# SDFIdk/malstroem

Measured on AMD Instinct MI355X. Metric: Mcells/s fill->D8->accum->label on 16384^2 f32 DEM, higher is better.
Workload: dtype f32 fill / f64 no-flats+D8+accum / u8 flowdir / i32 labels; 1 GPU; 16384x16384 float32 DEM (spectral fBm beta=2 seed 42 (SURVEY 8d recipe)): fill+depths -> no-flats fill -> D8 -> accumulation -> CCL+label_stats -> watersheds+label_count -> pour points; parallelism=1 GPU, one device context, fill_rounds=9, noflat_rounds=84, fill_tiles=70225, fill_visits=44601, fill_cycles=0, noflat_visits=411396, noflat_cycles=411396, nlabels=4637017, fill_algorithm=1, fill_launches=9, noflat_algorithm=2, pour_algorithm=1

## Files before the change

### malstroem_amd/csrc/watershed.hip

```cpp
#include <algorithm>

#include <type_traits>

#include "common.hpp"

namespace mh {
namespace {

constexpr int32_t NONE = 0x7fffffff;
constexpr uint32_t QFLAG = 0x80000000u, QMASK = 0x7fffffffu, QTERM = 0x7fffffffu;

__global__ __launch_bounds__(256) void ws_count_interior_nodir(const uint8_t *__restrict__ fd, int64_t H, int64_t W,
                                                              unsigned int *count)
{
    const int64_t i0 = ((int64_t)blockIdx.x * blockDim.x + threadIdx.x) * 16, n = H * W;
    unsigned hits = 0;
    if (i0 < n) {
        int64_t r = i0 / W, c = i0 - r * W;
        uint8_t b[16];
        const bool whole = i0 + 16 <= n;
        if (whole) {
            *reinterpret_cast<uint4 *>(b) = *reinterpret_cast<const uint4 *>(fd + i0);
        } else {
#pragma unroll
            for (int k = 0; k < 16; ++k) b[k] = i0 + k < n ? fd[i0 + k] : (uint8_t)0;
        }
#pragma unroll
        for (int k = 0; k < 16; ++k) {
            hits += (b[k] > 7u && r > 0 && r < H - 1 && c > 0 && c < W - 1) ? 1u : 0u;
            if (++c == W) {
                c = 0;
                ++r;
            }
        }
    }
#pragma unroll
    for (int o = 32; o > 0; o >>= 1) hits += __shfl_xor(hits, o);
    if (hits && (threadIdx.x & 63) == 0) atomicAdd(count, hits);
}

__global__ __launch_bounds__(256) void ws_init_kernel(const uint8_t *__restrict__ fd, const int32_t *__restrict__ lab,
                                                     int32_t *__restrict__ P, uint32_t *__restrict__ Q, int64_t H, int64_t W,
                                                     int32_t unassigned)
{
    const int64_t i = (int64_t)blockIdx.x * blockDim.x + threadIdx.x;
    if (i >= H * W) return;
    const int64_t d = downstream(fd, i, H, W);
    P[i] = lab[i] != unassigned ? (int32_t)i : (d < 0 ? NONE : (int32_t)d);
    if (Q) {
        const int64_t r = i / W, c = i - r * W;
        const bool edge = r == 0 || r == H - 1 || c == 0 || c == W - 1;
        Q[i] = (edge ? QFLAG : 0u) | (d < 0 ? QTERM : (uint32_t)d);
    }
}

constexpr int HOPS = 5;
constexpr int32_t DONE = (int32_t)0x80000000;
__global__ __launch_bounds__(256) void ws_jump_kernel(int32_t *P, uint32_t *Q, int64_t n, unsigned int *open)
{
    const int64_t i = (int64_t)blockIdx.x * blockDim.x + threadIdx.x;
    if (i >= n) return;
    bool ch = false;
    int32_t t = P[i];
    if (t >= 0 && t != NONE && t != (int32_t)i) {
        const int32_t t0 = t;
#pragma unroll
        for (int h = 0; h < HOPS; ++h) {
            const int32_t pt = P[t];
            if (pt == t) {
                t |= DONE;
                break;
            }
            t = pt;
            if (t < 0 || t == NONE) break;
        }
        if (t != t0) P[i] = t;
        ch = t >= 0 && t != NONE;
    }
    if (Q) {
        uint32_t q = Q[i];
        const uint32_t q0 = q;
#pragma unroll
        for (int h = 0; h < HOPS; ++h) {
            const uint32_t idx = q & QMASK;
            if (idx == QTERM) break;
            const uint32_t qt = Q[idx];
            q = ((q | qt) & QFLAG) | (qt & QMASK);
        }
        if (q != q0) Q[i] = q;
        ch |= (q & QMASK) != QTERM;
    }
    if (ch) *open = 1u;
}

constexpr int WT = WS_TILE;
__global__ __launch_bounds__(256) void ws_tile_kernel(const uint8_t *__restrict__ fd, const int32_t *__restrict__ lab, int32_t *__restrict__ P, int64_t H,
                                                     int64_t W, int ntc, int32_t unassigned, PourCandDev pc, int32_t *__restrict__ Pn)
{
    __shared__ uint16_t ptr[WT * WT];
    __shared__ uint8_t val[WT * WT];
    constexpr uint8_t V_LAB = 8, V_NONE = 9;
    const int ti = blockIdx.x / ntc, tj = blockIdx.x - ti * ntc;
    const int64_t r0 = (int64_t)ti * WT, c0 = (int64_t)tj * WT;
    const int lr = threadIdx.x >> 2, lc0 = (threadIdx.x & 3) * 16;
    const int64_t r = r0 + lr, cbase = c0 + lc0;
    const bool vec = (W & 15) == 0 && r < H && cbase + 16 <= W;
    uint8_t code[16];
    int32_t lb[16];
    if (vec) {
        const uint4 cv = *reinterpret_cast<const uint4 *>(fd + r * W + cbase);
        memcpy(code, &cv, 16);
#pragma unroll
        for (int q = 0; q < 4; ++q) {
            const int4 lv = *reinterpret_cast<const int4 *>(lab + r * W + cbase + 4 * q);
            lb[4 * q] = lv.x; lb[4 * q + 1] = lv.y; lb[4 * q + 2] = lv.z; lb[4 * q + 3] = lv.w;
        }
    } else {
#pragma unroll
        for (int k = 0; k < 16; ++k) {
            const bool in = r < H && cbase + k < W;
            code[k] = in ? fd[r * W + cbase + k] : (uint8_t)8;
            lb[k] = in ? lab[r * W + cbase + k] : unassigned;
        }
    }
    uint32_t lmask = 0;
    auto init_cells = [&](auto inner_tag) {
        constexpr bool INNER = decltype(inner_tag)::value;
#pragma unroll
        for (int k = 0; k < 16; ++k) {
            const int li = lr * WT + lc0 + k;
            const int64_t c = cbase + k;
            uint16_t p = (uint16_t)li;
            uint8_t v = V_NONE;
            if (INNER || (r < H && c < W)) {
                if (lb[k] != unassigned) {
                    lmask |= 1u << k;
                    v = V_LAB;
                } else if (code[k] <= 7u) {
                    const int lr2 = lr + dir_dr((int)code[k]), lc2 = lc0 + k + dir_dc((int)code[k]);
                    bool in_raster = true;
                    if (!INNER) {
                        const int64_t nr = r0 + lr2, nc = c0 + lc2;
                        in_raster = nr >= 0 && nr < H && nc >= 0 && nc < W;
                    }
                    if (in_raster) {
                        if (lr2 >= 0 && lr2 < WT && lc2 >= 0 && lc2 < WT) p = (uint16_t)(lr2 * WT + lc2);
                        else v = code[k];
                    }
                }
            }
            ptr[li] = p;
            val[li] = v;
        }
    };
    if (r0 > 0 && c0 > 0 && r0 + WT < H && c0 + WT < W) init_cells(std::true_type{});
    else init_cells(std::false_type{});
    __syncthreads();
    if (pc.mask0) {
        uint32_t cw[4] = {0x08080808u, 0x08080808u, 0x08080808u, 0x08080808u};
        if (vec) {
            const uint4 cv = *reinterpret_cast<const uint4 *>(fd + r * W + cbase);
            cw[0] = cv.x; cw[1] = cv.y; cw[2] = cv.z; cw[3] = cv.w;
        } else {
#pragma unroll
            for (int k = 0; k < 16; ++k)
                if (r < H && cbase + k < W) cw[k >> 2] = (cw[k >> 2] & ~(0xffu << (8 * (k & 3)))) | ((uint32_t)fd[r * W + cbase + k] << (8 * (k & 3)));
        }
        const uint32_t Wu = (uint32_t)W, Hu = (uint32_t)H, r0u = (uint32_t)r0, c0u = (uint32_t)c0;
        uint32_t m0 = 0, ml = 0;
#pragma unroll
        for (int k = 0; k < 16; ++k) {
            if (!(r < H && cbase + k < W)) continue;
            const unsigned cd = (cw[k >> 2] >> (8 * (k & 3))) & 0xffu;
            const bool mylab = (lmask >> k) & 1u;
            bool same = false;
            if (cd <= 7u) {
                const int lr2 = lr + dir_dr((int)cd), lc2 = lc0 + k + dir_dc((int)cd);
                const uint32_t nr = r0u + (uint32_t)lr2, nc = c0u + (uint32_t)lc2;
                if (nr < Hu && nc < Wu) {
                    const uint32_t gd = nr * Wu + nc;
                    bool labelled_d;
                    if (lr2 >= 0 && lr2 < WT && lc2 >= 0 && lc2 < WT) labelled_d = val[lr2 * WT + lc2] == V_LAB;
                    else labelled_d = lab[gd] != unassigned;
                    if (pc.components) same = labelled_d == mylab;
                    else same = (labelled_d ? lab[gd] : unassigned) == (mylab ? lab[(uint32_t)(r * W + cbase + k)] : unassigned);
                }
            }
            if (!same) {
                if (!mylab) m0 |= 1u << k;
                else ml |= 1u << k;
            }
        }
        pc.mask0[(int64_t)blockIdx.x * 256 + threadIdx.x] = (uint16_t)m0;
        __shared__ uint32_t wsum[4], base_s;
        const int lane = threadIdx.x & 63, wave = threadIdx.x >> 6;
        const uint32_t mine = (uint32_t)__builtin_popcount(ml);
        uint32_t incl = mine;
#pragma unroll
        for (int o = 1; o < 64; o <<= 1) {
            const uint32_t up = (uint32_t)__shfl_up((int)incl, o);
            if (lane >= o) incl += up;
        }
        if (lane == 63) wsum[wave] = incl;
        __syncthreads();
        if (threadIdx.x == 0) {
            const uint32_t tot = wsum[0] + wsum[1] + wsum[2] + wsum[3];
            const bool fits = tot <= POUR_TILE_CAP;
            if (!fits) pc.flags[0] = 1u;
            pc.tile_cnt[blockIdx.x] = fits ? tot : 0u;
            base_s = fits ? blockIdx.x * POUR_TILE_CAP : 0xffffffffu;
        }
        __syncthreads();
        if (base_s != 0xffffffffu) {
            uint32_t o = base_s + incl - mine;
            for (int w = 0; w < wave; ++w) o += wsum[w];
#pragma unroll
            for (int k = 0; k < 16; ++k)
                if ((ml >> k) & 1u) {
                    const uint32_t cell = (uint32_t)(r * W + cbase + k);
                    pc.list[o++] = make_uint2(cell, (uint32_t)lab[cell]);
                }
        }
    }
    for (int round = 0; round < 13; ++round) {
        bool ch = false;
#pragma unroll
        for (int k = 0; k < 16; ++k) {
            const int li = k * 256 + (int)threadIdx.x;
            const uint16_t p = ptr[li], q = ptr[p];
            if (q != p) {
                ptr[li] = q;
                ch = true;
            }
        }
        if (!__syncthreads_or(ch)) break;
    }
    int32_t out[16];
#pragma unroll
    for (int k = 0; k < 16; ++k) {
        const int li = lr * WT + lc0 + k;
        const int t = ptr[li];
        const int64_t gt = (r0 + (t >> 6)) * W + c0 + (t & 63);
        if (ptr[t] != t) out[k] = (int32_t)gt;
        else {
            const unsigned vb = val[t];
            int32_t v = NONE;
            if (vb == V_LAB) v = (int32_t)gt;
            else if (vb <= 7u) v = (int32_t)((r0 + (t >> 6) + dir_dr((int)vb)) * W + c0 + (t & 63) + dir_dc((int)vb));
            out[k] = (vb == V_LAB && t != li) ? (v | DONE) : v;
        }
        const int slot = ws_perim_slot(lr, lc0 + k);
        if (slot >= 0) Pn[(int64_t)blockIdx.x * 256 + slot] = (r < H && cbase + k < W) ? out[k] : NONE;
    }
    if (vec) {
#pragma unroll
        for (int q = 0; q < 4; ++q) *reinterpret_cast<int4 *>(P + r * W + cbase + 4 * q) = make_int4(out[4 * q], out[4 * q + 1], out[4 * q + 2], out[4 * q + 3]);
    } else {
#pragma unroll
        for (int k = 0; k < 16; ++k)
            if (r < H && cbase + k < W) P[r * W + cbase + k] = out[k];
    }
}

__global__ __launch_bounds__(256) void ws_jump_perimeter_kernel(int32_t *Pn, int64_t W, int ntc, int64_t nnodes, unsigned int *open)
{
    const int64_t x = (int64_t)blockIdx.x * blockDim.x + threadIdx.x;
    if (x >= nnodes || (x & 255) >= 4 * WT - 4) return;
    int32_t t = Pn[x];
    if (t < 0 || t == NONE) return;
    if (ws_node_of(t, (uint32_t)W, ntc) == x) return;
    const int32_t t0 = t;
#pragma unroll
    for (int h = 0; h < HOPS; ++h) {
        const int64_t nd = ws_node_of(t, (uint32_t)W, ntc);
        if (nd < 0) {
            if (t != t0) Pn[x] = t;
            return;
        }
        const int32_t pt = Pn[nd];
        if (pt == t) {
            t |= DONE;
            break;
        }
        t = pt;
        if (t < 0 || t == NONE) break;
    }
    if (t != t0) Pn[x] = t;
    if (t >= 0 && t != NONE) *open = 1u;
}

__global__ __launch_bounds__(256) void ws_assign_hop_kernel(const int32_t *__restrict__ P, const int32_t *__restrict__ Pn, const int32_t *src, int32_t *lab, int64_t n,
                                                           int64_t W, int ntc)
{
    const int64_t i0 = ((int64_t)blockIdx.x * blockDim.x + threadIdx.x) * 4;
    if (i0 >= n) return;
    const bool copy = src != lab;
    auto target = [&](int64_t i, int32_t p) -> int32_t {
        if (p == NONE || p == (int32_t)i) return -1;
        if (p >= 0) {
            const int64_t nd = ws_node_of(p, (uint32_t)W, ntc);
            if (nd < 0) return -1;
            const int32_t q = Pn[nd];
            if (q == p) p = q | DONE;
            else if (q < 0) p = q;
            else return -1;
        }
        return p & ~DONE;
    };
    if (i0 + 4 <= n && copy) {
        const int4 p4 = *reinterpret_cast<const int4 *>(P + i0);
        int4 v = *reinterpret_cast<const int4 *>(src + i0);
        const int32_t pq[4] = {p4.x, p4.y, p4.z, p4.w};
        int64_t nd[4];
        int32_t q[4], t[4];
#pragma unroll
        for (int k = 0; k < 4; ++k) {
            const bool hop = pq[k] >= 0 && pq[k] != NONE && pq[k] != (int32_t)(i0 + k);
            nd[k] = hop ? ws_node_of(pq[k], (uint32_t)W, ntc) : -1;
        }
#pragma unroll
        for (int k = 0; k < 4; ++k) q[k] = nd[k] >= 0 ? Pn[nd[k]] : NONE;
#pragma unroll
        for (int k = 0; k < 4; ++k) {
            int32_t pp = pq[k];
            t[k] = -1;
            if (pp == NONE || pp == (int32_t)(i0 + k)) continue;
            if (pp >= 0) {
                if (nd[k] < 0) continue;
                if (q[k] == pp) pp = q[k] | DONE;
                else if (q[k] < 0) pp = q[k];
                else continue;
            }
            t[k] = pp & ~DONE;
        }
        int32_t lv[4];
#pragma unroll
        for (int k = 0; k < 4; ++k) lv[k] = src[t[k] >= 0 ? t[k] : 0];
        if (t[0] >= 0) v.x = lv[0];
        if (t[1] >= 0) v.y = lv[1];
        if (t[2] >= 0) v.z = lv[2];
        if (t[3] >= 0) v.w = lv[3];
        *reinterpret_cast<int4 *>(lab + i0) = v;
    } else if (i0 + 4 <= n) {
        const int4 p = *reinterpret_cast<const int4 *>(P + i0);
        const int32_t t0 = target(i0, p.x), t1 = target(i0 + 1, p.y), t2 = target(i0 + 2, p.z), t3 = target(i0 + 3, p.w);
        if (copy) {
            int4 v = *reinterpret_cast<const int4 *>(src + i0);
            if (t0 >= 0) v.x = src[t0];
            if (t1 >= 0) v.y = src[t1];
            if (t2 >= 0) v.z = src[t2];
            if (t3 >= 0) v.w = src[t3];
            *reinterpret_cast<int4 *>(lab + i0) = v;
        } else {
            if (t0 >= 0) lab[i0] = src[t0];
            if (t1 >= 0) lab[i0 + 1] = src[t1];
            if (t2 >= 0) lab[i0 + 2] = src[t2];
            if (t3 >= 0) lab[i0 + 3] = src[t3];
        }
    } else {
        for (int64_t i = i0; i < n; ++i) {
            const int32_t t = target(i, P[i]);
            if (t >= 0) lab[i] = src[t];
            else if (copy) lab[i] = src[i];
        }
    }
}

__global__ __launch_bounds__(256) void ws_assign_kernel(const int32_t *__restrict__ P, const uint32_t *__restrict__ Q,
                                                       int32_t *lab, int64_t n, int32_t unassigned)
{
    const int64_t i = (int64_t)blockIdx.x * blockDim.x + threadIdx.x;
    if (i >= n) return;
    const int32_t p = P[i];
    if (p >= 0) return;
    const int32_t t = p & ~DONE;
    if (Q && !(Q[t] & QFLAG)) return;
    lab[i] = lab[t];
}

__global__ void ws_pseudo_kernel(int32_t *ws, int64_t H, int64_t W, int top, int bottom)
{
    const int64_t c = (int64_t)blockIdx.x * blockDim.x + threadIdx.x;
    if (c >= W) return;
    if (top) ws[c] = -(int32_t)(1 + c);
    if (bottom) ws[(H - 1) * W + c] = -(int32_t)(1 + W + c);
}
__global__ __launch_bounds__(256) void ws_root_labels_kernel(int32_t *out, int64_t H, int64_t W, int64_t row_off, int64_t Hg)
{
    const int64_t i = (int64_t)blockIdx.x * blockDim.x + threadIdx.x;
    if (i >= H * W) return;
    const int64_t r = i / W, c = i - r * W, gr = r + row_off;
    out[i] = (gr == 0 || gr == Hg - 1 || c == 0 || c == W - 1) ? BAND_ROOT : 0;
}
__global__ __launch_bounds__(256) void ws_hide_rootless_kernel(const int32_t *__restrict__ lab, const int32_t *__restrict__ rooted,
                                                              int32_t *__restrict__ out, int64_t n)
{
    const int64_t i = (int64_t)blockIdx.x * blockDim.x + threadIdx.x;
    if (i >= n) return;
    const int32_t l = lab[i];
    out[i] = (l == 0 || rooted[i] == BAND_ROOT) ? l : BAND_ROOTLESS;
}
__global__ __launch_bounds__(256) void ws_show_rootless_kernel(int32_t *__restrict__ ws, const int32_t *__restrict__ lab, int64_t n)
{
    const int64_t i = (int64_t)blockIdx.x * blockDim.x + threadIdx.x;
    if (i < n && ws[i] == BAND_ROOTLESS) ws[i] = lab[i];
}
__global__ __launch_bounds__(256) void ws_neg_lut_kernel(int32_t *lab, int64_t n, const int32_t *__restrict__ lut, int64_t nlut)
{
    const int64_t i0 = ((int64_t)blockIdx.x * blockDim.x + threadIdx.x) * 4;
    if (i0 >= n) return;
    auto look = [&](int32_t v) -> int32_t { return (v < 0 && (int64_t)(-(int64_t)v - 1) < nlut) ? lut[-(int64_t)v - 1] : v; };
    if (i0 + 4 <= n) {
        const int4 v = *reinterpret_cast<const int4 *>(lab + i0);
        if ((v.x | v.y | v.z | v.w) >= 0) return;
        *reinterpret_cast<int4 *>(lab + i0) = make_int4(look(v.x), look(v.y), look(v.z), look(v.w));
    } else {
        for (int64_t i = i0; i < n; ++i) lab[i] = look(lab[i]);
    }
}

}

int band_pseudo_labels_dev(int32_t *d_ws, int64_t H, int64_t W, int top, int bottom, hipStream_t s)
{
    hipLaunchKernelGGL(ws_pseudo_kernel, dim3((unsigned)cdiv(W, 256)), dim3(256), 0, s, d_ws, H, W, top, bottom);
    MH_HIP(hipGetLastError());
    return MHIP_OK;
}

int band_root_labels_dev(int32_t *d_out, int64_t H, int64_t W, int64_t row_off, int64_t Hg, hipStream_t s)
{
    hipLaunchKernelGGL(ws_root_labels_kernel, dim3((unsigned)cdiv(H * W, 256)), dim3(256), 0, s, d_out, H, W, row_off, Hg);
    MH_HIP(hipGetLastError());
    return MHIP_OK;
}

int band_hide_rootless_dev(const int32_t *d_lab, const int32_t *d_rooted, int32_t *d_out, int64_t n, hipStream_t s)
{
    hipLaunchKernelGGL(ws_hide_rootless_kernel, dim3((unsigned)cdiv(n, 256)), dim3(256), 0, s, d_lab, d_rooted, d_out, n);
    MH_HIP(hipGetLastError());
    return MHIP_OK;
}

int band_show_rootless_dev(int32_t *d_ws, const int32_t *d_lab, int64_t n, hipStream_t s)
{
    hipLaunchKernelGGL(ws_show_rootless_kernel, dim3((unsigned)cdiv(n, 256)), dim3(256), 0, s, d_ws, d_lab, n);
    MH_HIP(hipGetLastError());
    return MHIP_OK;
}

int negative_lut_dev(int32_t *d_lab, int64_t n, const int32_t *d_lut, int64_t nlut, hipStream_t s)
{
    hipLaunchKernelGGL(ws_neg_lut_kernel, dim3((unsigned)cdiv(cdiv(n, 4), 256)), dim3(256), 0, s, d_lab, n, d_lut, nlut);
    MH_HIP(hipGetLastError());
    return MHIP_OK;
}

namespace {
__global__ __launch_bounds__(1024) void pour_key0_kernel(const unsigned long long *__restrict__ tile_key0, int64_t ntiles, unsigned long long *key)
{
    unsigned long long best = 0;
    for (int64_t t = (int64_t)blockIdx.x * 1024 + threadIdx.x; t < ntiles; t += (int64_t)gridDim.x * 1024) best = tile_key0[t] > best ? tile_key0[t] : best;
#pragma unroll
    for (int o = 32; o > 0; o >>= 1) {
        const unsigned long long ob = __shfl_xor(best, o);
        best = ob > best ? ob : best;
    }
    if ((threadIdx.x & 63) == 0 && best) atomicMax(&key[0], best);
}

__global__ __launch_bounds__(256) void pour_finish_kernel(const unsigned long long *__restrict__ key, int64_t nrec, int64_t W, mhip_index_record *rec)
{
    const int64_t i = (int64_t)blockIdx.x * blockDim.x + threadIdx.x;
    if (i >= nrec) return;
    mhip_index_record r;
    const unsigned long long k = key[i];
    if (k == 0) {
        r.value = -__builtin_inf();
        r.row = -1;
        r.col = -1;
    } else {
        const uint64_t p = 0xffffffffu - (uint32_t)k;
        r.value = (double)(uint32_t)(k >> 32);
        r.row = (int64_t)(p / (uint64_t)W);
        r.col = (int64_t)(p % (uint64_t)W);
    }
    rec[i] = r;
}

}

int pour_finish_dev(unsigned long long *d_key, const unsigned long long *d_tile_key0, int64_t ntiles, int64_t nlab, int64_t W, mhip_index_record *d_rec,
                    hipStream_t s)
{
    hipLaunchKernelGGL(pour_key0_kernel, dim3((unsigned)std::min<int64_t>(cdiv(ntiles, 1024), 64)), dim3(1024), 0, s, d_tile_key0, ntiles, d_key);
    hipLaunchKernelGGL(pour_finish_kernel, dim3((unsigned)cdiv(nlab + 1, 256)), dim3(256), 0, s, d_key, nlab + 1, W, d_rec);
    MH_HIP(hipGetLastError());
    return MHIP_OK;
}

namespace {
struct PourNotify {
    PourLink *pl;
    bool done = false;
    void operator()(int v)
    {
        if (pl && pl->notify && !done) pl->notify(pl->arg, v);
        done = true;
    }
    ~PourNotify() { (*this)(0); }
};
}

int watersheds_dev(const uint8_t *d_fd, int32_t *d_labels, int64_t H, int64_t W, int32_t unassigned, hipStream_t s, bool band_mode,
                   const unsigned int *d_known_interior_nodir, const int32_t *d_src, PourLink *pour)
{
    PourNotify notify{pour};
    const int32_t *src = d_src ? d_src : d_labels;
    const int64_t n = H * W;
    if (n >= (int64_t)NONE - 1) {
        set_error("watersheds: %lld cells exceed the int32 index domain", (long long)n);
        return MHIP_ELIMIT;
    }
    const unsigned grid = (unsigned)cdiv(n, 256);
    DevBuf P, Q, flags;
    MH_TRY(P.alloc(4 * (size_t)n));
    MH_TRY(flags.alloc(sizeof(unsigned int) * 4));
    MH_HIP(hipMemsetAsync(flags.p, 0, sizeof(unsigned int) * 4, s));
    unsigned int *d_cnt = flags.as<unsigned int>(), *d_changed = d_cnt + 2;
    unsigned int interior_nodir = 0;
    if (!d_known_interior_nodir) hipLaunchKernelGGL(ws_count_interior_nodir, dim3((unsigned)cdiv(cdiv(n, 16), 256)), dim3(256), 0, s, d_fd, H, W, d_cnt);
    MH_HIP(hipMemcpyAsync(&interior_nodir, d_known_interior_nodir ? d_known_interior_nodir : d_cnt, 4, hipMemcpyDeviceToHost, s));
    MH_HIP(stream_sync(s));
    uint32_t *q = nullptr;
    if (interior_nodir && band_mode) {
        set_error("watersheds on a row band in one local pass need every flow path to leave the raster (interior NODIR cell found): "
                  "mhip_ctx_band_watershed_rooted takes any flow directions");
        return MHIP_EINVAL;
    }
    if (interior_nodir || (!d_known_interior_nodir && !band_mode)) {
        MH_TRY(Q.alloc(4 * (size_t)n));
        q = Q.as<uint32_t>();
    }
    if (!q) {
        const int64_t ntr = cdiv(H, WT), ntc = cdiv(W, WT), ntiles = ntr * ntc;
        const bool cand = pour && pour->dev.mask0 && unassigned == 0 && n < 0xffffffffll;
        DevBuf Pn;
        MH_TRY(Pn.alloc(4 * 256 * (size_t)ntiles));
        hipLaunchKernelGGL(ws_tile_kernel, dim3((unsigned)ntiles), dim3(256), 0, s, d_fd, src, P.as<int32_t>(), H, W, (int)ntc, unassigned,
                           cand ? pour->dev : PourCandDev(), Pn.as<int32_t>());
        if (cand) {
            MH_HIP(hipEventRecord(pour->ev, s));
            notify(1);
        } else {
            notify(0);
        }
        constexpr int MAX_ROUNDS = 40;
        for (int round = 0; round < MAX_ROUNDS;) {
            const int k = round == 0 ? 2 : 1;
            MH_HIP(hipMemsetAsync(d_changed, 0, 8, s));
            for (int j = 0; j < k; ++j)
                hipLaunchKernelGGL(ws_jump_perimeter_kernel, dim3((unsigned)ntiles), dim3(256), 0, s, Pn.as<int32_t>(), W, (int)ntc, ntiles * 256, d_changed + j);
            unsigned int h[2] = {0, 0};
            MH_HIP(hipMemcpyAsync(h, d_changed, 8, hipMemcpyDeviceToHost, s));
            MH_HIP(stream_sync(s));
            round += k;
            if (!h[k - 1]) break;
        }
        hipLaunchKernelGGL(ws_assign_hop_kernel, dim3((unsigned)cdiv(cdiv(n, 4), 256)), dim3(256), 0, s, P.as<int32_t>(), Pn.as<int32_t>(), src, d_labels, n, W,
                           (int)ntc);
        MH_HIP(hipGetLastError());
        MH_HIP(stream_sync(s));
        return MHIP_OK;
    }
    if (src != d_labels) MH_HIP(hipMemcpyAsync(d_labels, src, 4 * (size_t)n, hipMemcpyDeviceToDevice, s));
    hipLaunchKernelGGL(ws_init_kernel, dim3(grid), dim3(256), 0, s, d_fd, d_labels, P.as<int32_t>(), q, H, W, unassigned);
    constexpr int MAX_ROUNDS = 32;
    for (int round = 0; round < MAX_ROUNDS;) {
        const int k = round == 0 ? 2 : 1;
        MH_HIP(hipMemsetAsync(d_changed, 0, 8, s));
        for (int j = 0; j < k; ++j)
            hipLaunchKernelGGL(ws_jump_kernel, dim3(grid), dim3(256), 0, s, P.as<int32_t>(), q, n, d_changed + j);
        unsigned int h[2] = {0, 0};
        MH_HIP(hipMemcpyAsync(h, d_changed, 8, hipMemcpyDeviceToHost, s));
        MH_HIP(stream_sync(s));
        round += k;
        if (!h[k - 1]) break;
    }
    hipLaunchKernelGGL(ws_assign_kernel, dim3(grid), dim3(256), 0, s, P.as<int32_t>(), q, d_labels, n, unassigned);
    MH_HIP(hipGetLastError());
    MH_HIP(stream_sync(s));
    return MHIP_OK;
}

}
```

Measured before the change: 12350 Mcells/s.

## Restructure watershed tile kernel: byte-offset pointers, bitmask pour test, active-set jumping

Rewrites the per-tile watershed kernel so shared pointers are stored as byte offsets. Interior tiles now initialise with vectorised LDS stores, using a perm-based direction decode. Pour-candidate detection for interior tiles uses per-row label bitmasks kept in shared memory instead of per-cell neighbour lookups. Pointer jumping tracks active cells in registers and skips settled halves, and the output stage uses mul24 and vectorised perimeter writes. The aim is to cut LDS and global traffic and per-cell branching in one stage of the pipeline, at the cost of much more intricate code and risk of edge-case bugs (perimeter layout, Pn slots for out-of-range cells).

```diff
diff --git a/malstroem_amd/csrc/watershed.hip b/malstroem_amd/csrc/watershed.hip
--- a/malstroem_amd/csrc/watershed.hip
+++ b/malstroem_amd/csrc/watershed.hip
@@ -97,8 +97,8 @@
 __global__ __launch_bounds__(256) void ws_tile_kernel(const uint8_t *__restrict__ fd, const int32_t *__restrict__ lab, int32_t *__restrict__ P, int64_t H,
                                                      int64_t W, int ntc, int32_t unassigned, PourCandDev pc, int32_t *__restrict__ Pn)
 {
-    __shared__ uint16_t ptr[WT * WT];
-    __shared__ uint8_t val[WT * WT];
+    __shared__ __attribute__((aligned(16))) uint16_t ptr[WT * WT];
+    __shared__ __attribute__((aligned(16))) uint8_t val[WT * WT];
     constexpr uint8_t V_LAB = 8, V_NONE = 9;
     const int ti = blockIdx.x / ntc, tj = blockIdx.x - ti * ntc;
     const int64_t r0 = (int64_t)ti * WT, c0 = (int64_t)tj * WT;
@@ -124,27 +124,22 @@
         }
     }
     uint32_t lmask = 0;
-    auto init_cells = [&](auto inner_tag) {
-        constexpr bool INNER = decltype(inner_tag)::value;
+    auto init_border = [&]() {
 #pragma unroll
         for (int k = 0; k < 16; ++k) {
             const int li = lr * WT + lc0 + k;
             const int64_t c = cbase + k;
-            uint16_t p = (uint16_t)li;
+            uint16_t p = (uint16_t)(2 * li);
             uint8_t v = V_NONE;
-            if (INNER || (r < H && c < W)) {
+            if (r < H && c < W) {
                 if (lb[k] != unassigned) {
                     lmask |= 1u << k;
                     v = V_LAB;
                 } else if (code[k] <= 7u) {
                     const int lr2 = lr + dir_dr((int)code[k]), lc2 = lc0 + k + dir_dc((int)code[k]);
-                    bool in_raster = true;
-                    if (!INNER) {
-                        const int64_t nr = r0 + lr2, nc = c0 + lc2;
-                        in_raster = nr >= 0 && nr < H && nc >= 0 && nc < W;
-                    }
-                    if (in_raster) {
-                        if (lr2 >= 0 && lr2 < WT && lc2 >= 0 && lc2 < WT) p = (uint16_t)(lr2 * WT + lc2);
+                    const int64_t nr = r0 + lr2, nc = c0 + lc2;
+                    if (nr >= 0 && nr < H && nc >= 0 && nc < W) {
+                        if (lr2 >= 0 && lr2 < WT && lc2 >= 0 && lc2 < WT) p = (uint16_t)(2 * (lr2 * WT + lc2));
                         else v = code[k];
                     }
                 }
@@ -153,8 +148,38 @@
             val[li] = v;
         }
     };
-    if (r0 > 0 && c0 > 0 && r0 + WT < H && c0 + WT < W) init_cells(std::true_type{});
-    else init_cells(std::false_type{});
+    auto init_inner = [&]() {
+        uint32_t cwi[4];
+        memcpy(cwi, code, 16);
+        const int li0 = lr * WT + lc0;
+        uint16_t pl[16];
+        uint8_t vl[16];
+#pragma unroll
+        for (int k = 0; k < 16; ++k) {
+            const uint32_t d4 = __builtin_amdgcn_perm(0xbfff3f40u, 0x4101c1c0u, cwi[k >> 2]);
+            const uint32_t cd = code[k];
+            const int32_t n2 = 2 * (li0 + k + (int32_t)(int8_t)(d4 >> (8 * (k & 3))));
+            bool leaves = (uint32_t)n2 >= 2u * WT * WT;
+            if (k == 0) leaves |= lc0 == 0 && ((0xe0u >> (cd & 7u)) & 1u);
+            if (k == 15) leaves |= lc0 == WT - 16 && ((0x0eu >> (cd & 7u)) & 1u);
+            const bool labelled = lb[k] != unassigned, flows = !labelled && cd <= 7u;
+            lmask |= labelled ? 1u << k : 0u;
+            pl[k] = (uint16_t)(flows && !leaves ? n2 : 2 * (li0 + k));
+            vl[k] = labelled ? V_LAB : (flows && leaves ? (uint8_t)cd : V_NONE);
+        }
+        uint4 pa, pb, va;
+        memcpy(&pa, pl, 16);
+        memcpy(&pb, pl + 8, 16);
+        memcpy(&va, vl, 16);
+        *reinterpret_cast<uint4 *>(ptr + li0) = pa;
+        *reinterpret_cast<uint4 *>(ptr + li0 + 8) = pb;
+        *reinterpret_cast<uint4 *>(val + li0) = va;
+    };
+    __shared__ uint64_t lrow[WT];
+    const bool inner = r0 > 0 && c0 > 0 && r0 + WT < H && c0 + WT < W;
+    if (inner) init_inner();
+    else init_border();
+    reinterpret_cast<uint16_t *>(lrow)[threadIdx.x] = (uint16_t)lmask;
     __syncthreads();
     if (pc.mask0) {
         uint32_t cw[4] = {0x08080808u, 0x08080808u, 0x08080808u, 0x08080808u};
@@ -168,27 +193,64 @@
         }
         const uint32_t Wu = (uint32_t)W, Hu = (uint32_t)H, r0u = (uint32_t)r0, c0u = (uint32_t)c0;
         uint32_t m0 = 0, ml = 0;
-#pragma unroll
-        for (int k = 0; k < 16; ++k) {
-            if (!(r < H && cbase + k < W)) continue;
-            const unsigned cd = (cw[k >> 2] >> (8 * (k & 3))) & 0xffu;
-            const bool mylab = (lmask >> k) & 1u;
-            bool same = false;
-            if (cd <= 7u) {
-                const int lr2 = lr + dir_dr((int)cd), lc2 = lc0 + k + dir_dc((int)cd);
-                const uint32_t nr = r0u + (uint32_t)lr2, nc = c0u + (uint32_t)lc2;
-                if (nr < Hu && nc < Wu) {
-                    const uint32_t gd = nr * Wu + nc;
-                    bool labelled_d;
-                    if (lr2 >= 0 && lr2 < WT && lc2 >= 0 && lc2 < WT) labelled_d = val[lr2 * WT + lc2] == V_LAB;
-                    else labelled_d = lab[gd] != unassigned;
-                    if (pc.components) same = labelled_d == mylab;
-                    else same = (labelled_d ? lab[gd] : unassigned) == (mylab ? lab[(uint32_t)(r * W + cbase + k)] : unassigned);
+        if (inner && pc.components) {
+            auto rowbits = [&](uint64_t x) -> uint64_t {
+                uint64_t z = (x << 1) >> lc0;
+                if (lc0 == 48) z |= (x >> 63) << 16;
+                return z & 0x3ffffull;
+            };
+            const uint64_t win = (lr > 0 ? rowbits(lrow[lr > 0 ? lr - 1 : 0]) : 0ull) | (rowbits(lrow[lr]) << 18) |
+                                 ((lr < WT - 1 ? rowbits(lrow[lr < WT - 1 ? lr + 1 : lr]) : 0ull) << 36);
+            const uint64_t ow = (lr == 0 ? 0x3ffffull : 0ull) | (lr == WT - 1 ? 0x3ffffull << 36 : 0ull) |
+                                (lc0 == 0 ? (1ull | 1ull << 18 | 1ull << 36) : 0ull) | (lc0 == 48 ? (1ull << 17 | 1ull << 35 | 1ull << 53) : 0ull);
+            uint32_t ld = 0, ot = 0, nodir = 0;
+#pragma unroll
+            for (int q = 0; q < 4; ++q) {
+                const uint32_t o4 = __builtin_amdgcn_perm(0x00122425u, 0x26140201u, cw[q]);
+#pragma unroll
+                for (int j = 0; j < 4; ++j) {
+                    const int k = 4 * q + j;
+                    const uint32_t s = (o4 >> (8 * j)) & 0x3fu;
+                    ld |= (uint32_t)(win >> s) & (1u << k);
+                    ot |= (uint32_t)(ow >> s) & (1u << k);
+                    nodir |= ((cw[q] >> (8 * j)) & 0xffu) > 7u ? 1u << k : 0u;
                 }
             }
-            if (!same) {
-                if (!mylab) m0 |= 1u << k;
-                else ml |= 1u << k;
+            ot &= ~nodir;
+            uint32_t cand = ((ld ^ lmask) | nodir) & ~ot & 0xffffu;
+            const uint32_t cell0 = (uint32_t)(r * W + cbase);
+#pragma unroll
+            for (int k = 0; k < 16; ++k)
+                if ((ot >> k) & 1u) {
+                    const int cd = (int)((cw[k >> 2] >> (8 * (k & 3))) & 0xffu);
+                    const uint32_t gd = cell0 + (uint32_t)k + (uint32_t)dir_dr(cd) * Wu + (uint32_t)dir_dc(cd);
+                    if ((lab[gd] != unassigned) != (bool)((lmask >> k) & 1u)) cand |= 1u << k;
+                }
+            m0 = cand & ~lmask;
+            ml = cand & lmask;
+        } else {
+#pragma unroll
+            for (int k = 0; k < 16; ++k) {
+                if (!(r < H && cbase + k < W)) continue;
+                const unsigned cd = (cw[k >> 2] >> (8 * (k & 3))) & 0xffu;
+                const bool mylab = (lmask >> k) & 1u;
+                bool same = false;
+                if (cd <= 7u) {
+                    const int lr2 = lr + dir_dr((int)cd), lc2 = lc0 + k + dir_dc((int)cd);
+                    const uint32_t nr = r0u + (uint32_t)lr2, nc = c0u + (uint32_t)lc2;
+                    if (nr < Hu && nc < Wu) {
+                        const uint32_t gd = nr * Wu + nc;
+                        bool labelled_d;
+                        if (lr2 >= 0 && lr2 < WT && lc2 >= 0 && lc2 < WT) labelled_d = val[lr2 * WT + lc2] == V_LAB;
+                        else labelled_d = lab[gd] != unassigned;
+                        if (pc.components) same = labelled_d == mylab;
+                        else same = (labelled_d ? lab[gd] : unassigned) == (mylab ? lab[(uint32_t)(r * W + cbase + k)] : unassigned);
+                    }
+                }
+                if (!same) {
+                    if (!mylab) m0 |= 1u << k;
+                    else ml |= 1u << k;
+                }
             }
         }
         pc.mask0[(int64_t)blockIdx.x * 256 + threadIdx.x] = (uint16_t)m0;
@@ -222,35 +284,90 @@
                 }
         }
     }
+    auto at = [&](int32_t byte_off) -> uint16_t & { return *reinterpret_cast<uint16_t *>(reinterpret_cast<char *>(ptr) + byte_off); };
+    int32_t pw[16];
+    bool act[2] = {false, false};
+#pragma unroll
+    for (int k = 0; k < 16; ++k) {
+        const int32_t own = 2 * (k * 256 + (int)threadIdx.x), p = ptr[k * 256 + (int)threadIdx.x];
+        pw[k] = p != own ? p : -1;
+        act[k >> 3] |= p != own;
+    }
+    bool capped = true;
     for (int round = 0; round < 13; ++round) {
-        bool ch = false;
+#pragma unroll
+        for (int h = 0; h < 2; ++h) {
+            if (!act[h]) continue;
+            bool moved = false;
+            int32_t qq[8];
+#pragma unroll
+            for (int j = 0; j < 8; ++j) {
+                qq[j] = pw[8 * h + j];
+                if (pw[8 * h + j] >= 0) qq[j] = at(pw[8 * h + j]);
+            }
+#pragma unroll
+            for (int j = 0; j < 8; ++j) {
+                const int k = 8 * h + j;
+                if (qq[j] != pw[k]) {
+                    ptr[k * 256 + (int)threadIdx.x] = (uint16_t)qq[j];
+                    pw[k] = qq[j];
+                    moved = true;
+                } else {
+                    pw[k] = -1;
+                }
+            }
+            act[h] = moved;
+        }
+        if (!__syncthreads_or(act[0] || act[1])) {
+            capped = false;
+            break;
+        }
+    }
+    const uint32_t Wu = (uint32_t)W, tile0 = (uint32_t)r0 * Wu + (uint32_t)c0;
+    int32_t out[16];
+    auto write_out = [&](auto w24_tag) {
+        constexpr bool W24 = decltype(w24_tag)::value;
+        auto mulw = [&](uint32_t x, uint32_t w) -> uint32_t { return W24 ? (uint32_t)__mul24((int)x, (int)w) : x * w; };
+        const int li0 = lr * WT + lc0;
+        uint32_t tw[8];
+        {
+            const uint4 a = *reinterpret_cast<const uint4 *>(ptr + li0), b = *reinterpret_cast<const uint4 *>(ptr + li0 + 8);
+            tw[0] = a.x; tw[1] = a.y; tw[2] = a.z; tw[3] = a.w; tw[4] = b.x; tw[5] = b.y; tw[6] = b.z; tw[7] = b.w;
+        }
+        uint32_t cyc = 0;
+        if (capped) {
+#pragma unroll
+            for (int k = 0; k < 16; ++k) {
+                const int32_t t2 = (int32_t)((tw[k >> 1] >> (16 * (k & 1))) & 0xffffu);
+                if (at(t2) != t2) cyc |= 1u << k;
+            }
+        }
+        uint32_t vb[16];
+#pragma unroll
+        for (int k = 0; k < 16; ++k) vb[k] = val[((tw[k >> 1] >> (16 * (k & 1))) & 0xffffu) >> 1];
 #pragma unroll
         for (int k = 0; k < 16; ++k) {
-            const int li = k * 256 + (int)threadIdx.x;
-            const uint16_t p = ptr[li], q = ptr[p];
-            if (q != p) {
-                ptr[li] = q;
-                ch = true;
-            }
-        }
-        if (!__syncthreads_or(ch)) break;
-    }
-    int32_t out[16];
-#pragma unroll
-    for (int k = 0; k < 16; ++k) {
-        const int li = lr * WT + lc0 + k;
-        const int t = ptr[li];
-        const int64_t gt = (r0 + (t >> 6)) * W + c0 + (t & 63);
-        if (ptr[t] != t) out[k] = (int32_t)gt;
-        else {
-            const unsigned vb = val[t];
-            int32_t v = NONE;
-            if (vb == V_LAB) v = (int32_t)gt;
-            else if (vb <= 7u) v = (int32_t)((r0 + (t >> 6) + dir_dr((int)vb)) * W + c0 + (t & 63) + dir_dc((int)vb));
-            out[k] = (vb == V_LAB && t != li) ? (v | DONE) : v;
-        }
-        const int slot = ws_perim_slot(lr, lc0 + k);
-        if (slot >= 0) Pn[(int64_t)blockIdx.x * 256 + slot] = (r < H && cbase + k < W) ? out[k] : NONE;
+            const uint32_t t = ((tw[k >> 1] >> (16 * (k & 1))) & 0xffffu) >> 1;
+            const uint32_t gt = tile0 + t + mulw(t >> 6, Wu - 64u);
+            const uint32_t e = __builtin_amdgcn_perm(0x00102021u, 0x22120201u, vb[k]);
+            const uint32_t entry = gt - Wu - 1u + mulw((e >> 4) & 3u, Wu) + (e & 3u);
+            int32_t v = vb[k] <= 7u ? (int32_t)entry : NONE;
+            if (vb[k] == V_LAB) v = t != (uint32_t)(li0 + k) ? (int32_t)(gt | (uint32_t)DONE) : (int32_t)gt;
+            out[k] = (cyc >> k) & 1u ? (int32_t)gt : v;
+        }
+    };
+    if (Wu < (1u << 23)) write_out(std::true_type{});
+    else write_out(std::false_type{});
+    {
+        int32_t *pn = Pn + (int64_t)blockIdx.x * 256;
+        if (lr == 0 || lr == WT - 1) {
+#pragma unroll
+            for (int q = 0; q < 4; ++q)
+                *reinterpret_cast<int4 *>(pn + (lr == 0 ? 0 : WT) + lc0 + 4 * q) = make_int4(out[4 * q], out[4 * q + 1], out[4 * q + 2], out[4 * q + 3]);
+        } else {
+            if (lc0 == 0) pn[2 * WT + (lr - 1)] = out[0];
+            if (lc0 == WT - 16) pn[2 * WT + (WT - 2) + (lr - 1)] = out[15];
+        }
     }
     if (vec) {
 #pragma unroll
```

After: 12450 Mcells/s (median of 6 runs). Within noise of the previous version (+0.8%).
